# GuildOfWeavers/genSTARK

Measured on AMD Instinct MI355X. Metric: prove() ms + NTT GF(p) elements/sec, MiMC-128 2^20 steps, higher is better.
Workload: dtype u128; 1 GPU; MiMC-128 prove(), 2^20 steps, extensionFactor 16, exeQueryCount 48, friQueryCount 64, blake2s256; one independent proof per GPU; evaluation_domain=16777216, ntt_points_per_prove=17827072, ntt_transforms_per_prove=4, proof_bytes=371695

## Files before the change

genstark_amd/csrc/air_mimc.hip:

```cpp
#include "common.h"
#include "host_field.h"

__global__ void k_mimc_constraints(const fe *__restrict__ p, uint64_t nc, uint64_t shift, const fe *__restrict__ k, uint64_t klen,
                                   fe *__restrict__ out) {
    for (uint64_t j = blockIdx.x * (uint64_t)blockDim.x + threadIdx.x; j < nc; j += (uint64_t)gridDim.x * blockDim.x) {
        uint64_t jn = j + shift;
        if (jn >= nc) jn -= nc;
        fe x = p[j], nx = p[jn];
        fe x3 = fe_mul(fe_mul(x, x), x);
        out[j] = fe_sub(nx, fe_add(x3, k[j % klen]));
    }
}

#define GS_MIMC_COMP_MAX_PERIOD 32
#define GS_MIMC_COMP_MAX_ROOTS 4
struct MimcCompArgs {
    fe qz[GS_MIMC_COMP_MAX_PERIOD];
    fe bt[GS_MIMC_COMP_MAX_PERIOD];
    fe lt[GS_MIMC_COMP_MAX_PERIOD];
    fe ipoly[GS_MIMC_COMP_MAX_ROOTS];
    uint64_t root[GS_MIMC_COMP_MAX_ROOTS];
    fe x_last;
};
__global__ void k_mimc_composition(const fe *__restrict__ p, uint64_t n, uint64_t shift, const fe *__restrict__ k, uint64_t klen,
                                   const fe *__restrict__ tw_lo, const fe *__restrict__ tw_hi, int log_lo, int logn, const fe *__restrict__ u,
                                   MimcCompArgs a, uint32_t period, uint32_t nroots, int with_lc, fe *__restrict__ out) {
    __shared__ fe qz[GS_MIMC_COMP_MAX_PERIOD], bt[GS_MIMC_COMP_MAX_PERIOD], lt[GS_MIMC_COMP_MAX_PERIOD];
    if (threadIdx.x < period) { qz[threadIdx.x] = a.qz[threadIdx.x]; bt[threadIdx.x] = a.bt[threadIdx.x]; lt[threadIdx.x] = a.lt[threadIdx.x]; }
    __syncthreads();
    for (uint64_t i = blockIdx.x * (uint64_t)blockDim.x + threadIdx.x; i < n; i += (uint64_t)gridDim.x * blockDim.x) {
        fe x = tw_lo[i & ((1ull << log_lo) - 1)];
        if (logn > log_lo) x = fe_mul(x, tw_hi[i >> log_lo]);
        const fe pi = p[i], pn = p[(i + shift) & (n - 1)];
        const fe q = fe_sub(pn, fe_add(fe_mul(fe_mul(pi, pi), pi), k[i % klen]));
        const fe d = fe_mul(fe_mul(q, fe_sub(x, a.x_last)), qz[i & (period - 1)]);
        fe iv = a.ipoly[nroots - 1];
        for (int c = (int)nroots - 2; c >= 0; c--) iv = fe_add(fe_mul(iv, x), a.ipoly[c]);
        fe b = fe_mul(fe_sub(pi, iv), bt[i & (period - 1)]);
        for (uint32_t r = 0; r < nroots; r++) b = fe_mul(b, u[(i + n - a.root[r]) & (n - 1)]);
        fe r = fe_add(d, b);
        if (with_lc) r = fe_add(r, fe_mul(pi, lt[i & (period - 1)]));
        out[i] = r;
    }
}

#define GS_MIMC_CHUNK_BODY(STEP)                                                                                \
    for (uint64_t i = base; i < end; i++) {                                                                    \
        t[i] = hf_mimc_out(x);                                      \
        x = STEP(x, rc[ri]);                                   \
        if (++ri == nrc) ri = 0;                                                                               \
    }                                                                                                          \
    *ri_io = ri;                                                                                               \
    return x;
static hfe mimc_chunk_generic(hfe *t, hfe x, const hfe *rc, uint32_t nrc, uint32_t *ri_io, uint64_t base, uint64_t end) {
    uint32_t ri = *ri_io;
    GS_MIMC_CHUNK_BODY(hf_mimc_step_weak)
}
#if defined(__x86_64__) && !defined(__HIP_DEVICE_COMPILE__) && !defined(GS_SMALL_Q) && !defined(GS_WIDE_BITS)
#define GS_MIMC_CHUNK_V3 1
__attribute__((target("arch=x86-64-v3,tune=znver5"))) static hfe mimc_chunk_v3(hfe *t, hfe x, const hfe *rc, uint32_t nrc, uint32_t *ri_io, uint64_t base,
                                                                               uint64_t end) {
    uint32_t ri = *ri_io;
    GS_MIMC_CHUNK_BODY(hf_cube_add_rows)
}
#endif
extern "C" {

int gs_mimc_trace(gs_ctx *c, const gs_elt *seed, const uint8_t *rc_host, uint32_t nrc, uint64_t steps, void *out) {
    if (!c || !seed || !rc_host || !out) return GS_ERR_ARG;
    if (!nrc || !steps) return gs_fail(c, GS_ERR_ARG, "mimc_trace: empty");
    std::vector<hfe> rc(nrc);
    for (uint32_t i = 0; i < nrc; i++) rc[i] = hf_load(rc_host + GS_ELT * i);
    int rcode = gs_trace_begin(c, steps * GS_ELT);
    if (rcode) return rcode;
    hfe *t = (hfe *)c->h_trace;
    hfe x = hf_load(seed);
    uint32_t ri = 0;
    const uint64_t CHUNK = 1ull << 16;
#ifdef GS_MIMC_CHUNK_V3
    static const bool v3 = __builtin_cpu_supports("avx2") && __builtin_cpu_supports("bmi2") && __builtin_cpu_supports("fma");
#else
    const bool v3 = false;
#endif
    for (uint64_t base = 0; base < steps; base += CHUNK) {
        const uint64_t end = base + CHUNK < steps ? base + CHUNK : steps;
#ifdef GS_MIMC_CHUNK_V3
        if (v3) x = mimc_chunk_v3(t, x, rc.data(), nrc, &ri, base, end);
        else
#endif
            x = mimc_chunk_generic(t, x, rc.data(), nrc, &ri, base, end);
        (void)v3;
        GS_HIP(c, hipMemcpyAsync((uint8_t *)out + base * GS_ELT, t + base, (end - base) * GS_ELT, hipMemcpyHostToDevice, c->stream));
    }
    return gs_trace_end(c);
}

int gs_mimc_constraints(gs_ctx *c, const void *p_comp, uint64_t nc, uint64_t shift, const void *k_table, uint64_t klen, void *out) {
    if (!c || !p_comp || !k_table || !out) return GS_ERR_ARG;
    if (!nc || !klen) return gs_fail(c, GS_ERR_ARG, "mimc_constraints: empty");
    hipLaunchKernelGGL(k_mimc_constraints, dim3(gs_grid(nc)), dim3(256), 0, c->stream, (const fe *)p_comp, nc, shift % nc,
                       (const fe *)k_table, klen, (fe *)out);
    GS_LAUNCH_CHECK(c);
    return GS_OK;
}

int gs_mimc_composition(gs_ctx *c, const void *p_eval, uint64_t n, uint64_t steps, const gs_elt *omega, const void *k_table, uint64_t klen,
                        const uint8_t *coeffs_host, uint64_t q_inc, uint64_t b_inc, const uint8_t *ipoly_host, const uint64_t *root_index_host,
                        uint32_t nroots, const uint8_t *lc_coeffs_host, void *out) {
    if (!c || !p_eval || !omega || !k_table || !coeffs_host || !ipoly_host || !root_index_host || !out) return GS_ERR_ARG;
    if (!gs_is_pow2(n) || !gs_is_pow2(steps) || steps > n || !klen) return gs_fail(c, GS_ERR_ARG, "mimc_composition: bad sizes");
    const uint64_t period = n / steps;
    if (period > GS_MIMC_COMP_MAX_PERIOD || nroots == 0 || nroots > GS_MIMC_COMP_MAX_ROOTS)
        return gs_fail(c, GS_ERR_UNSUPPORTED, "mimc_composition: n / steps <= %d and 1..%d assertions", GS_MIMC_COMP_MAX_PERIOD, GS_MIMC_COMP_MAX_ROOTS);
    if (q_inc % steps || b_inc % steps) return gs_fail(c, GS_ERR_ARG, "mimc_composition: degree increments must be multiples of the trace length");
    const fe w = fe_from_bytes(omega);
    const fe *lo, *hi, *u;
    int log_lo;
    int rc = gs_plan_pow_tables(c, w, n, &lo, &hi, &log_lo);
    if (!rc) rc = gs_plan_inverse_table(c, w, n, &u);
    if (rc) return rc;
    const fe d0 = fe_from_bytes(coeffs_host), d1 = fe_from_bytes(coeffs_host + GS_ELT), b0 = fe_from_bytes(coeffs_host + 2 * GS_ELT),
             b1 = fe_from_bytes(coeffs_host + 3 * GS_ELT);
    const fe l0 = lc_coeffs_host ? fe_from_bytes(lc_coeffs_host) : fe_zero(), l1 = lc_coeffs_host ? fe_from_bytes(lc_coeffs_host + GS_ELT) : fe_zero();
    MimcCompArgs a;
    uint64_t ksum = 0;
    for (uint32_t r = 0; r < GS_MIMC_COMP_MAX_ROOTS; r++) {
        a.root[r] = r < nroots ? root_index_host[r] & (n - 1) : 0;
        a.ipoly[r] = r < nroots ? fe_from_bytes(ipoly_host + GS_ELT * r) : fe_zero();
        if (r < nroots) ksum = (ksum + a.root[r]) & (n - 1);
    }
    const fe scale = gs_memo_pow(c, w, (n - ksum) & (n - 1));
    const std::vector<fe> &tab = gs_memo(c, gs_memo_key("mimc_comp").add(w).add(n).add(steps).add(q_inc).add(b_inc), [&](std::vector<fe> &t) {
        const fe g = fe_pow_u64(w, steps);
        const fe gq = fe_pow_u64(g, (q_inc / steps) % period), gb = fe_pow_u64(g, (b_inc / steps) % period);
        fe gj = fe_one(), gqj = fe_one(), gbj = fe_one();
        for (uint64_t j = 0; j < period; j++) {
            t.push_back(fe_inv(fe_sub(gj, fe_one())));
            t.push_back(gqj);
            t.push_back(gbj);
            gj = fe_mul(gj, g); gqj = fe_mul(gqj, gq); gbj = fe_mul(gbj, gb);
        }
        t.push_back(fe_pow_u64(w, (steps - 1) * period));
    });
    for (uint64_t j = 0; j < GS_MIMC_COMP_MAX_PERIOD; j++) {
        if (j < period) {
            a.qz[j] = fe_mul(fe_add(d0, fe_mul(d1, tab[3 * j + 1])), tab[3 * j]);
            a.bt[j] = fe_mul(fe_add(b0, fe_mul(b1, tab[3 * j + 2])), scale);
            a.lt[j] = fe_add(l0, fe_mul(l1, tab[3 * j + 2]));
        } else {
            a.qz[j] = a.bt[j] = a.lt[j] = fe_zero();
        }
    }
    a.x_last = tab[3 * period];
    gs_traffic(c, 2 * n * GS_ELT, n, "k_mimc_composition");
    hipLaunchKernelGGL(k_mimc_composition, dim3(gs_grid(n)), dim3(256), 0, c->stream, (const fe *)p_eval, n, period, (const fe *)k_table, klen, lo, hi,
                       log_lo, gs_log2(n), u, a, (uint32_t)period, nroots, lc_coeffs_host ? 1 : 0, (fe *)out);
    GS_LAUNCH_CHECK(c);
    return GS_OK;
}

}
```

genstark_amd/csrc/common.h:

```cpp
#pragma once
#include <hip/hip_runtime.h>
#include <stdint.h>
#include <stdio.h>
#include <stdarg.h>
#include <string.h>

#include <array>

#include <map>
#include <mutex>
#include <string>
#include <vector>

#include "../../include/gstark.h"
#if defined(GS_SMALL_Q)
#include "gf_small.h"
#elif defined(GS_WIDE_BITS)
#include "gf_wide.h"
#else
#include "gf128.h"
#endif

#if defined(GF_RUNTIME_MODULUS)
typedef int (*gs_rt_push_fn)(void);
// ... 61 lines not shown
    int up_half = 0;
    hipEvent_t up_done[2] = {};
    bool up_pending[2] = {false, false};
};

int gs_fail(gs_ctx *c, int code, const char *fmt, ...);

static inline void gs_traffic(gs_ctx *c, uint64_t bytes, uint64_t units, const char *fmt, ...) __attribute__((format(printf, 4, 5)));
static inline void gs_traffic(gs_ctx *c, uint64_t bytes, uint64_t units, const char *fmt, ...) {
    if (!c->traffic_on) return;
    char name[64];
    va_list ap;
    va_start(ap, fmt);
    vsnprintf(name, sizeof name, fmt, ap);
    va_end(ap);
    auto &e = c->traffic[name];
    e[0] += 1; e[1] += bytes; e[2] += units;
}

struct gs_memo_key {
    std::string k;
    explicit gs_memo_key(const char *tag) : k(tag) {}
    gs_memo_key &add(const void *p, size_t n) { k.append((const char *)p, n); return *this; }
    gs_memo_key &add(uint64_t v) { return add(&v, sizeof v); }
    gs_memo_key &add(const fe &v) { return add(&v, sizeof v); }
};
template <class Build>
static inline const std::vector<fe> &gs_memo(gs_ctx *c, const gs_memo_key &key, Build build) {
    auto it = c->scalar_memo.find(key.k);
    if (it == c->scalar_memo.end()) {
        if (c->scalar_memo.size() > 1024) c->scalar_memo.clear();
        it = c->scalar_memo.emplace(key.k, std::vector<fe>()).first;
        build(it->second);
    }
    return it->second;
}
static inline fe gs_memo_pow(gs_ctx *c, const fe &w, uint64_t e) {
    return gs_memo(c, gs_memo_key("pow").add(w).add(e), [&](std::vector<fe> &t) { t.push_back(fe_pow_u64(w, e)); })[0];
}

#define GS_HIP(c, call)                                                                              \
    do {                                                                                             \
        hipError_t e_ = (call);                                                                      \
        if (e_ != hipSuccess) return gs_fail((c), GS_ERR_DEVICE, "%s: %s", #call, hipGetErrorString(e_)); \
    } while (0)

#define GS_LAUNCH_CHECK(c) GS_HIP(c, hipGetLastError())

static inline bool gs_is_pow2(uint64_t x) { return x && !(x & (x - 1)); }
static inline int gs_log2(uint64_t x) { int l = 0; while ((1ull << l) < x) l++; return l; }

static inline fe fe_from_bytes(const uint8_t *b) { fe r; memcpy(&r, b, sizeof(fe)); return r; }
static inline void fe_to_bytes(uint8_t *b, const fe &v) { memcpy(b, &v, sizeof(fe)); }
static inline fe fe_from_u64(uint64_t v) { return fe_make((uint32_t)v, (uint32_t)(v >> 32), 0, 0); }

int gs_stage_reserve(gs_ctx *c, uint64_t bytes);
int gs_defer_flush(gs_ctx *c);
int gs_push_reserve(gs_ctx *c, uint64_t bytes, void **host);
int gs_push_commit(gs_ctx *c, void *dst, const void *host, uint64_t bytes);
int gs_push(gs_ctx *c, void *dst, const void *host_src, uint64_t bytes);
int gs_readback_reserve(gs_ctx *c, uint32_t bytes, void **slot_dev, unsigned long long **flag_dev, unsigned long long *value, uint64_t *ticket);
int gs_trace_begin(gs_ctx *c, uint64_t bytes);
int gs_trace_end(gs_ctx *c);
int gs_tmp_alloc(gs_ctx *c, uint64_t bytes, void **p);
void gs_tmp_free(gs_ctx *c, void *p);

static inline unsigned gs_grid(uint64_t work_items, unsigned block = 256, unsigned cap = 256 * 8) {
    uint64_t g = (work_items + block - 1) / block;
    if (g < 1) g = 1;
    if (g > cap) g = cap;
    return (unsigned)g;
}

int gs_jit_trace_segments(gs_ctx *c, const uint32_t *code, uint32_t ninstr, const uint32_t *icode, uint32_t init_ninstr, const uint8_t *consts_host,
                          uint32_t nconsts, uint32_t vm_regs, uint32_t registers, const uint64_t *soff, const uint64_t *slen, const uint8_t *statics_host,
                          uint32_t nstatic, const fe *dconst, const fe *dstat, const fe *drows, uint64_t segments, uint64_t seglen, fe *out);
int gs_jit_constraints(gs_ctx *c, const uint32_t *code, uint32_t ninstr, const uint8_t *consts_host, uint32_t nconsts, uint32_t vm_regs,
                       uint32_t registers, const uint64_t *soff, const uint64_t *slen, const fe *dconst, const fe *p, uint64_t nc, uint64_t shift,
                       const fe *statics, fe *out, uint64_t prow, uint64_t pstride);

void gs_plans_destroy(gs_ctx *c);
int gs_plan_pow_tables(gs_ctx *c, const fe &omega, uint64_t n, const fe **tw_lo, const fe **tw_hi, int *log_lo);
int gs_plan_inverse_table(gs_ctx *c, const fe &omega, uint64_t n, const fe **u);
int gs_plan_inverse_table_shifted(gs_ctx *c, const fe &omega, uint64_t n, const fe &shift, const fe **u);
```

genstark_amd/csrc/hash.hip:

```cpp
#include "common.h"

#include "hash_core.h"

template <int ALG, typename Loader>
__device__ __forceinline__ void digest_words16(Loader word16, uint32_t nwords16, uint32_t out[8]) {
    const uint32_t len = nwords16 * 16;
    if (ALG == 1) {
        uint32_t h[8] = {0x6A09E667u ^ 0x01010020u, 0xBB67AE85u, 0x3C6EF372u, 0xA54FF53Au,
                         0x510E527Fu, 0x9B05688Cu, 0x1F83D9ABu, 0x5BE0CD19u};
        const uint32_t nblocks = nwords16 ? (nwords16 + 3) / 4 : 1;
        for (uint32_t blk = 0; blk < nblocks; blk++) {
            uint32_t m[16];
#pragma unroll
            for (int q = 0; q < 4; q++) {
                uint32_t wi = blk * 4 + q;
                uint4 x = wi < nwords16 ? word16(wi) : make_uint4(0, 0, 0, 0);
                m[4 * q] = x.x; m[4 * q + 1] = x.y; m[4 * q + 2] = x.z; m[4 * q + 3] = x.w;
            }
            const bool last = blk == nblocks - 1;
            b2s_compress(h, m, last ? len : (blk + 1) * 64, last);
        }
#pragma unroll
        for (int i = 0; i < 8; i++) out[i] = h[i];
    } else {
// ... 10 lines not shown
                w[4 * q] = bswap32(x.x); w[4 * q + 1] = bswap32(x.y); w[4 * q + 2] = bswap32(x.z); w[4 * q + 3] = bswap32(x.w);
            }
            if (blk == nblocks - 1) { w[14] = 0; w[15] = len * 8; }
            sha256_compress(h, w);
        }
#pragma unroll
        for (int i = 0; i < 8; i++) out[i] = bswap32(h[i]);
    }
}

__device__ __forceinline__ void store_digest(uint4 *out, uint64_t i, const uint32_t d[8]) {
    out[2 * i] = make_uint4(d[0], d[1], d[2], d[3]);
    out[2 * i + 1] = make_uint4(d[4], d[5], d[6], d[7]);
}

struct HashPtrArgs {
    const uint4 *v[GS_MAX_COMBINE];
};

template <int ALG>
__global__ void k_hash_merge_rows(HashPtrArgs va, uint32_t count, uint64_t n, uint4 *__restrict__ out) {
    for (uint64_t i = blockIdx.x * (uint64_t)blockDim.x + threadIdx.x; i < n; i += (uint64_t)gridDim.x * blockDim.x) {
        uint32_t d[8];
        digest_words16<ALG>([&](uint32_t w) { return va.v[w / GS_EW][i * GS_EW + w % GS_EW]; }, count * GS_EW, d);
        store_digest(out, i, d);
    }
}
template <int ALG>
__global__ void k_hash_merge_rows_table(const uint4 *const *__restrict__ tab, uint32_t count, uint64_t n, uint4 *__restrict__ out) {
    for (uint64_t i = blockIdx.x * (uint64_t)blockDim.x + threadIdx.x; i < n; i += (uint64_t)gridDim.x * blockDim.x) {
        uint32_t d[8];
        digest_words16<ALG>([&](uint32_t w) { return tab[w / GS_EW][i * GS_EW + w % GS_EW]; }, count * GS_EW, d);
        store_digest(out, i, d);
    }
}
template <int ALG>
__global__ void k_hash_merge_rows1(const uint4 *__restrict__ v, uint64_t n, uint4 *__restrict__ out) {
    for (uint64_t i = blockIdx.x * (uint64_t)blockDim.x + threadIdx.x; i < n; i += (uint64_t)gridDim.x * blockDim.x) {
        uint32_t d[8];
        digest_words16<ALG>([&](uint32_t w) { return v[i * GS_EW + w]; }, GS_EW, d);
        store_digest(out, i, d);
    }
}
template <int ALG>
__global__ void k_hash_values(const uint4 *__restrict__ buf, uint32_t w16, uint64_t count, uint4 *__restrict__ out) {
    for (uint64_t i = blockIdx.x * (uint64_t)blockDim.x + threadIdx.x; i < count; i += (uint64_t)gridDim.x * blockDim.x) {
        const uint4 *p = buf + i * w16;
        uint32_t d[8];
        digest_words16<ALG>([&](uint32_t w) { return p[w]; }, w16, d);
        store_digest(out, i, d);
    }
}
template <int ALG>
__global__ void k_hash_values64(const uint4 *__restrict__ buf, uint64_t count, uint4 *__restrict__ out) {
    for (uint64_t i = blockIdx.x * (uint64_t)blockDim.x + threadIdx.x; i < count; i += (uint64_t)gridDim.x * blockDim.x) {
        const uint4 *p = buf + i * 4;
        uint4 x0 = p[0], x1 = p[1], x2 = p[2], x3 = p[3];
        uint32_t d[8];
        digest_words16<ALG>([&](uint32_t w) { return w == 0 ? x0 : (w == 1 ? x1 : (w == 2 ? x2 : x3)); }, 4, d);
        store_digest(out, i, d);
    }
}
template <int ALG, int SRC>
__device__ __forceinline__ void first_layer_digest(const HashPtrArgs &va, uint32_t count, const uint4 *__restrict__ child, uint64_t i, uint32_t d[8]) {
    if constexpr (SRC == 0) {
        const uint4 *p = child + 4 * i;
        const uint4 x0 = p[0], x1 = p[1], x2 = p[2], x3 = p[3];
        digest_words16<ALG>([&](uint32_t w) { return w == 0 ? x0 : (w == 1 ? x1 : (w == 2 ? x2 : x3)); }, 4, d);
    } else if constexpr (SRC == 1) {
        const uint4 *p = va.v[0] + i * GS_EW;
        digest_words16<ALG>([&](uint32_t w) { return p[w]; }, GS_EW, d);
    } else {
        digest_words16<ALG>([&](uint32_t w) { return va.v[w / GS_EW][i * GS_EW + w % GS_EW]; }, count * GS_EW, d);
    }
}
template <int ALG>
__device__ __forceinline__ void merge_digests(const uint32_t l[8], const uint32_t r[8], uint32_t d[8]) {
    const uint4 x0 = make_uint4(l[0], l[1], l[2], l[3]), x1 = make_uint4(l[4], l[5], l[6], l[7]);
    const uint4 x2 = make_uint4(r[0], r[1], r[2], r[3]), x3 = make_uint4(r[4], r[5], r[6], r[7]);
    digest_words16<ALG>([&](uint32_t w) { return w == 0 ? x0 : (w == 1 ? x1 : (w == 2 ? x2 : x3)); }, 4, d);
}

#define GS_MERKLE_MAX_LV 4
template <int ALG, int SRC>
__global__ __launch_bounds__(256) void k_merkle_fused(HashPtrArgs va, uint32_t count, const uint4 *__restrict__ child, uint64_t groups, int lv,
                                                      uint4 *__restrict__ outA, uint4 *__restrict__ nodes, uint64_t wA) {
    __shared__ uint32_t pending[GS_MERKLE_MAX_LV - 1][8][256];
    const int K = 1 << (lv - 1), tid = threadIdx.x;
    for (uint64_t g = blockIdx.x * (uint64_t)256 + tid; g < groups; g += (uint64_t)gridDim.x * 256) {
        for (int k = 0; k < K; k++) {
            uint64_t idx = g * K + k;
            uint32_t cur[8];
            first_layer_digest<ALG, SRC>(va, count, child, idx, cur);
            store_digest(outA, idx, cur);
            int h = 0;
            for (; (k >> h) & 1; h++) {
                uint32_t l[8];
#pragma unroll
                for (int w = 0; w < 8; w++) l[w] = pending[h][w][tid];
                merge_digests<ALG>(l, cur, cur);
                idx >>= 1;
                store_digest(nodes, (wA >> (h + 1)) + idx, cur);
            }
            if (h < lv - 1) {
#pragma unroll
                for (int w = 0; w < 8; w++) pending[h][w][tid] = cur[w];
            }
        }
    }
}

struct RootTail {
    uint4 *slot;
    unsigned long long *flag;
    unsigned long long value;
    fe *point;
};
__device__ __forceinline__ fe prng_point(const uint32_t *seed);

#define GS_MERKLE_CHUNK 1024
#define GS_MERKLE_SUBTREE_THREADS 1024
template <int ALG>
__device__ __forceinline__ void subtree_levels(uint4 *sh, uint32_t first_m, uint64_t wl, uint64_t offset, uint4 *__restrict__ nodes) {
    for (uint32_t m = first_m; m >= 1; m >>= 1, wl >>= 1) {
        bool done = false;
        if constexpr (ALG == 1) {
            if (m <= blockDim.x / 4) {
                if (threadIdx.x < 4 * m) {
                    const uint32_t i = threadIdx.x >> 2, l = threadIdx.x & 3u, s = m + i;
                    uint32_t *w = reinterpret_cast<uint32_t *>(sh);
                    uint32_t lo, hi;
                    b2s_node_quad(w + 16 * s, (int)l, lo, hi);
                    w[8 * s + l] = lo;
                    w[8 * s + 4 + l] = hi;
                    uint32_t *g = reinterpret_cast<uint32_t *>(nodes) + 8 * (wl + offset * m + i);
                    g[l] = lo;
                    g[4 + l] = hi;
                }
                done = true;
            }
        }
        if (!done) {
            for (uint32_t i = threadIdx.x; i < m; i += blockDim.x) {
                const uint32_t s = m + i;
                const uint4 x0 = sh[4 * s], x1 = sh[4 * s + 1], x2 = sh[4 * s + 2], x3 = sh[4 * s + 3];
                uint32_t d[8];
                digest_words16<ALG>([&](uint32_t k) { return k == 0 ? x0 : (k == 1 ? x1 : (k == 2 ? x2 : x3)); }, 4, d);
                sh[2 * s] = make_uint4(d[0], d[1], d[2], d[3]);
                sh[2 * s + 1] = make_uint4(d[4], d[5], d[6], d[7]);
                store_digest(nodes, wl + offset * m + i, d);
            }
        }
        __syncthreads();
    }
}

template <int ALG, int SRC>
__global__ __launch_bounds__(GS_MERKLE_SUBTREE_THREADS) void k_merkle_subtree(HashPtrArgs va, uint32_t count, const uint4 *__restrict__ layerA, uint4 *__restrict__ outA,
                                                        uint4 *__restrict__ nodes, uint64_t wA, uint32_t chunk, RootTail tail, unsigned int *counter) {
    __shared__ uint4 sh[4 * GS_MERKLE_CHUNK];
    const uint64_t base = (uint64_t)blockIdx.x * chunk;
    for (uint32_t i = threadIdx.x; i < chunk; i += blockDim.x) {
        if constexpr (SRC == 0) {
            sh[2 * (chunk + i)] = layerA[2 * (base + i)];
            sh[2 * (chunk + i) + 1] = layerA[2 * (base + i) + 1];
        } else {
            uint32_t d[8];
            first_layer_digest<ALG, SRC>(va, count, nullptr, base + i, d);
            store_digest(outA, base + i, d);
            sh[2 * (chunk + i)] = make_uint4(d[0], d[1], d[2], d[3]);
            sh[2 * (chunk + i) + 1] = make_uint4(d[4], d[5], d[6], d[7]);
        }
    }
    __syncthreads();
    subtree_levels<ALG>(sh, chunk / 2, wA >> 1, blockIdx.x, nodes);
    bool at_root = chunk == wA;
    if (counter && gridDim.x > 1) {
        __shared__ int last_sh;
        const uint32_t G = gridDim.x;
        if (threadIdx.x == 0) {
            __threadfence();
            last_sh = atomicAdd(counter, 1u) == G - 1;
            if (last_sh) __threadfence();
        }
        __syncthreads();
        if (!last_sh) return;
        for (uint32_t i = threadIdx.x; i < G; i += blockDim.x) {
            sh[2 * (G + i)] = nodes[2 * (G + (uint64_t)i)];
            sh[2 * (G + i) + 1] = nodes[2 * (G + (uint64_t)i) + 1];
        }
        if (threadIdx.x == 0) atomicExch(counter, 0u);
        __syncthreads();
        subtree_levels<ALG>(sh, G / 2, G >> 1, 0, nodes);
        at_root = true;
    }
    if (at_root && threadIdx.x == 0) {
        nodes[0] = make_uint4(0, 0, 0, 0);
        nodes[1] = make_uint4(0, 0, 0, 0);
        if (tail.slot) {
            tail.slot[0] = sh[2];
            tail.slot[1] = sh[3];
            __threadfence_system();
            __hip_atomic_store(tail.flag, tail.value, __ATOMIC_RELEASE, __HIP_MEMORY_SCOPE_SYSTEM);
        }
        if (tail.point) {
            const uint4 r0 = sh[2], r1 = sh[3];
            const uint32_t seed[8] = {r0.x, r0.y, r0.z, r0.w, r1.x, r1.y, r1.z, r1.w};
            *tail.point = prng_point(seed);
        }
    }
}

#define GS_FRI_MAX_LAYERS 16
static int arrival_counters(gs_ctx *c, unsigned int **counters) {
    if (!c->fri_points) {
        int rc = gs_alloc(c, (GS_FRI_MAX_LAYERS + 1) * GS_ELT + 64, &c->fri_points);
        if (rc) return rc;
        GS_HIP(c, hipMemsetAsync((uint8_t *)c->fri_points + (GS_FRI_MAX_LAYERS + 1) * GS_ELT, 0, 64, c->stream));
    }
    *counters = (unsigned int *)((uint8_t *)c->fri_points + (GS_FRI_MAX_LAYERS + 1) * GS_ELT);
    return GS_OK;
}

static inline uint64_t hash_blocks(int alg, uint64_t bytes) { return alg == 1 ? (bytes + 63) / 64 : (bytes + 9 + 63) / 64; }
#define GS_MERKLE_SUBW (1ull << 15)
template <int ALG>
static int merkle_run(gs_ctx *c, int src, const HashPtrArgs &va, uint32_t count, const void *leaves_in, void *leaves_out, uint64_t n, uint4 *nd,
                      const RootTail *root_tail = nullptr) {
    const RootTail none = {nullptr, nullptr, 0, nullptr};
    auto tail_for = [&](uint64_t width, uint32_t chunk) { return root_tail && (width == chunk || width / chunk <= GS_MERKLE_CHUNK) ? *root_tail : none; };
    const uint32_t CHUNK_X = 256;
    unsigned int *counters = nullptr;
    if (n > CHUNK_X) {
        int rc = arrival_counters(c, &counters);
        if (rc) return rc;
        counters += 1;
    }
    const dim3 blk(256), sub_blk(GS_MERKLE_SUBTREE_THREADS);
    uint64_t w = n;
    const uint4 *cur = (const uint4 *)leaves_in;
    if (src != 0) {
        uint4 *lo = (uint4 *)leaves_out;
        if (n > GS_MERKLE_SUBW) {
            int lv = 1;
            const int maxlv = src == 2 ? 2 : GS_MERKLE_MAX_LV;
            while (lv < maxlv && (n >> lv) >= GS_MERKLE_SUBW) lv++;
            const uint64_t groups = n >> (lv - 1);
            {
                const uint64_t above = n - (n >> (lv - 1));
                gs_traffic(c, n * ((uint64_t)count * GS_ELT + 32) + above * 32, n * hash_blocks(ALG, (uint64_t)count * GS_ELT) + above, "k_merkle_fused<%d, %d>", ALG, src);
            }
            if (src == 1) hipLaunchKernelGGL((k_merkle_fused<ALG, 1>), dim3(gs_grid(groups)), blk, 0, c->stream, va, count, nullptr, groups, lv, lo, nd, n);
            else hipLaunchKernelGGL((k_merkle_fused<ALG, 2>), dim3(gs_grid(groups)), blk, 0, c->stream, va, count, nullptr, groups, lv, lo, nd, n);
            w = n >> (lv - 1);
            cur = lv == 1 ? lo : nd + 2 * w;
        } else {
            const uint32_t chunk = (uint32_t)(n <= CHUNK_X ? n : CHUNK_X);
            gs_traffic(c, n * ((uint64_t)count * GS_ELT + 32) + n * 32, n * hash_blocks(ALG, (uint64_t)count * GS_ELT) + n - 1, "k_merkle_subtree<%d, %d>", ALG, src);
            if (src == 1) hipLaunchKernelGGL((k_merkle_subtree<ALG, 1>), dim3((unsigned)(n / chunk)), sub_blk, 0, c->stream, va, count, nullptr, lo, nd, n, chunk, tail_for(n, chunk), counters);
            else hipLaunchKernelGGL((k_merkle_subtree<ALG, 2>), dim3((unsigned)(n / chunk)), sub_blk, 0, c->stream, va, count, nullptr, lo, nd, n, chunk, tail_for(n, chunk), counters);
            GS_LAUNCH_CHECK(c);
            return GS_OK;
        }
    }
    while (w > GS_MERKLE_SUBW) {
        int lv = 1;
        while (lv < GS_MERKLE_MAX_LV && (w >> (lv + 1)) >= GS_MERKLE_SUBW) lv++;
#ifdef GS_NTT_EXPERIMENTS
        if (const char *e = getenv("GSTARK_MERKLE_NODE_MIN_GROUPS")) {
            const int K = atoi(e);
            lv = 1;
            while (lv < GS_MERKLE_MAX_LV && (w >> (lv + 1)) >= GS_MERKLE_SUBW) lv++;
            while (lv > 1 && (w >> lv) < (1ull << K)) lv--;
        }
#endif
        const uint64_t groups = w >> lv;
        gs_traffic(c, w * 32 + (w - (w >> lv)) * 32, w - (w >> lv), "k_merkle_fused<%d, 0>", ALG);
        hipLaunchKernelGGL((k_merkle_fused<ALG, 0>), dim3(gs_grid(groups)), blk, 0, c->stream, va, 0u, cur, groups, lv, nd + 2 * (w / 2), nd, w / 2);
        w >>= lv;
        cur = nd + 2 * w;
    }
    while (w > 1) {
        const uint32_t chunk = (uint32_t)(w <= CHUNK_X ? w : (w / CHUNK_X <= GS_MERKLE_CHUNK ? CHUNK_X : GS_MERKLE_CHUNK));
        gs_traffic(c, w * 32 + (w - 1) * 32, w - 1, "k_merkle_subtree<%d, 0>", ALG);
        hipLaunchKernelGGL((k_merkle_subtree<ALG, 0>), dim3((unsigned)(w / chunk)), sub_blk, 0, c->stream, va, 0u, cur, nullptr, nd, w, chunk, tail_for(w, chunk), counters);
        w /= chunk;
        cur = nd + 2 * w;
        if (counters && w <= GS_MERKLE_CHUNK) break;
    }
    GS_LAUNCH_CHECK(c);
    return GS_OK;
}

template <int ALG>
static int hash_values_launch(gs_ctx *c, const void *buf, uint64_t value_size, uint64_t count, void *out) {
    if (!count) return GS_OK;
    if (value_size == 64)
        hipLaunchKernelGGL(k_hash_values64<ALG>, dim3(gs_grid(count)), dim3(256), 0, c->stream, (const uint4 *)buf, count, (uint4 *)out);
    else
        hipLaunchKernelGGL(k_hash_values<ALG>, dim3(gs_grid(count)), dim3(256), 0, c->stream, (const uint4 *)buf,
                           (uint32_t)(value_size / 16), count, (uint4 *)out);
    GS_LAUNCH_CHECK(c);
    return GS_OK;
}

static int check_alg(gs_ctx *c, gs_hash_alg alg) {
    if (alg != GS_HASH_SHA256 && alg != GS_HASH_BLAKE2S256) return gs_fail(c, GS_ERR_ARG, "unknown hash algorithm %d", (int)alg);
    return GS_OK;
}

__device__ __forceinline__ fe prng_point(const uint32_t *seed);
__global__ void k_prng_point(const uint32_t *__restrict__ seed, fe *__restrict__ out) {
    if (threadIdx.x || blockIdx.x) return;
    *out = prng_point(seed);
}
__device__ __forceinline__ fe prng_point(const uint32_t *seed) {
    uint32_t h[8] = {0x6a09e667u, 0xbb67ae85u, 0x3c6ef372u, 0xa54ff53au, 0x510e527fu, 0x9b05688cu, 0x1f83d9abu, 0x5be0cd19u};
    uint32_t w[16];
#pragma unroll
    for (int i = 0; i < 8; i++) w[i] = bswap32(seed[i]);
    w[8] = 0x80000000u;
#pragma unroll
    for (int i = 9; i < 15; i++) w[i] = 0;
    w[15] = 256;
    sha256_compress(h, w);
#if !defined(GS_SMALL_Q) && !defined(GS_WIDE_BITS)
    const uint32_t r[8] = {h[7], h[6], h[5], h[4], h[3], h[2], h[1], h[0]};
    return fe_reduce_wide(r);
#else
    fe x = fe_zero();
    const fe b = fe_make(256u, 0u, 0u, 0u);
    for (int i = 0; i < 8; i++)
        for (int k = 3; k >= 0; k--) x = fe_add(fe_mul(x, b), fe_make((h[i] >> (8 * k)) & 0xFFu, 0u, 0u, 0u));
    return x;
#endif
}
int gs_prng_point_dev(gs_ctx *c, const void *seed32_dev, fe *out_dev) {
    if (((uintptr_t)seed32_dev) & 3) return gs_fail(c, GS_ERR_ARG, "prng_point: the seed must be 4-byte aligned");
    hipLaunchKernelGGL(k_prng_point, dim3(1), dim3(64), 0, c->stream, (const uint32_t *)seed32_dev, out_dev);
    GS_LAUNCH_CHECK(c);
    return GS_OK;
}


#define GS_FRI_CH 256
#define GS_FRI_THREADS (4 * GS_FRI_CH)
#define GS_FRI_ONE_LAUNCH_LEAVES (1ull << 15)
struct FriLayerDesc {
    const fe *column;
    fe *next;
    uint4 *leaves, *nodes;
    fe *point_out;
    uint4 *slot;
    unsigned long long *flag;
    unsigned long long value;
    uint64_t rows, step;
};
struct FriLayersArgs {
    FriLayerDesc layer[GS_FRI_MAX_LAYERS];
    uint32_t first, count;
    const fe *point_in;
// ... 301 lines not shown
```

genstark_amd/csrc/ntt.hip:

```cpp
#include <stdlib.h>

#include "common.h"

#if !defined(GS_SMALL_Q) && !defined(GS_WIDE_BITS)
#define GS_NTT_LAZY 1
#include "gf128_lazy.h"
struct alignas(32) lz8 { int32_t l[8]; };
#endif

struct NttPlan {
    fe omega;
    uint64_t n = 0;
    int logn = 0, log_lo = 0;
    fe *tw_lo = nullptr;
    fe *tw_hi = nullptr;
    int npass = 0;
    int L[4] = {0, 0, 0, 0};
    fe *wR[4] = {nullptr, nullptr, nullptr, nullptr};
    fe *twp[4] = {nullptr, nullptr, nullptr, nullptr};
    fe w16[8];
    fe *inv_table = nullptr;
    std::map<std::string, fe *> inv_table_shifted;
#ifdef GS_NTT_LAZY
    lzw *wtab = nullptr;
// ... 645 lines not shown
    }
    if (p->logn >= 8) {
        int np = (p->logn + 7) / 8, base = p->logn / np, extra = p->logn % np;
        p->npass = np;
        fe w16 = fe_pow_u64(omega, n / 16), cur = fe_one();
        for (int i = 0; i < 8; i++) { p->w16[i] = cur; cur = fe_mul(cur, w16); }
#ifdef GS_NTT_LAZY
        {
            lzw host[8];
            for (int i = 1; i < 8; i++) lz_wform(p->w16[i], host[i - 1]);
            lz_wform(fe_inv(fe_from_u64(n)), host[7]);
            if ((rc = gs_alloc(c, sizeof host, &q))) { delete p; return rc; }
            p->wtab = (lzw *)q;
            if (hipMemcpyAsync(p->wtab, host, sizeof host, hipMemcpyHostToDevice, c->stream) != hipSuccess ||
                hipStreamSynchronize(c->stream) != hipSuccess) {
                delete p;
                return gs_fail(c, GS_ERR_DEVICE, "ntt: twiddle upload failed");
            }
        }
#endif
#ifdef GS_NTT_LAZY
        if ((rc = gs_alloc(c, (1ull << p->log_lo) * GS_ELT, &q))) { delete p; return rc; }
        p->tw_loR = (fe *)q;
        hipLaunchKernelGGL(k_scale_table, dim3(gs_grid(1ull << p->log_lo)), dim3(256), 0, c->stream, p->tw_lo, p->tw_loR, 1ull << p->log_lo, lz_mont_r());
#endif
        uint64_t Ns_acc = 1;
        for (int i = 0; i < np; i++) {
            p->L[i] = base + (i < extra ? 1 : 0);
            uint64_t R = 1ull << p->L[i];
            if (i > 0 && Ns_acc * R <= max_pass_twiddle_entries()) {
#if !defined(GS_NTT_LAZY) || defined(GS_NTT_EXPERIMENTS)
                if ((rc = gs_alloc(c, Ns_acc * R * GS_ELT, &q))) { delete p; return rc; }
                p->twp[i] = (fe *)q;
                hipLaunchKernelGGL(k_build_pass_twiddles, dim3(gs_grid(Ns_acc * R)), dim3(256), 0, c->stream, p->twp[i], Ns_acc, R,
                                   n / (Ns_acc * R), p->tw_lo, p->tw_hi, p->log_lo, p->logn, fe_one(), 0);
#endif
#ifdef GS_NTT_LAZY
                if ((rc = gs_alloc(c, Ns_acc * R * GS_ELT, &q))) { delete p; return rc; }
                p->twpR[i] = (fe *)q;
                hipLaunchKernelGGL(k_build_pass_twiddles, dim3(gs_grid(Ns_acc * R)), dim3(256), 0, c->stream, p->twpR[i], Ns_acc, R,
                                   n / (Ns_acc * R), p->tw_lo, p->tw_hi, p->log_lo, p->logn, lz_mont_r(), 1);
#endif
            }
            Ns_acc *= R;
            if (R > 16) {
                for (int k = 0; k < i; k++)
                    if (p->L[k] == p->L[i]) p->wR[i] = p->wR[k];
                if (!p->wR[i]) {
                    if ((rc = gs_alloc(c, R * GS_ELT, &q))) { delete p; return rc; }
                    p->wR[i] = (fe *)q;
                    if ((rc = gs_power_series_dev(c, fe_pow_u64(omega, n / R), R, p->wR[i]))) { delete p; return rc; }
                }
#ifdef GS_NTT_LAZY
                for (int k = 0; k < i; k++)
                    if (p->L[k] == p->L[i]) p->wRz[i] = p->wRz[k];
                if (!p->wRz[i]) {
                    if ((rc = gs_alloc(c, R * sizeof(lz8), &q))) { delete p; return rc; }
                    p->wRz[i] = (lz8 *)q;
                    hipLaunchKernelGGL(k_build_lz_table, dim3(gs_grid(R)), dim3(256), 0, c->stream, p->wR[i], p->wRz[i], R, lz_mont_r(), 1);
                }
#endif
            }
        }
    }
    c->plans[key] = p;
    *out = p;
    return GS_OK;
}

void gs_plans_destroy(gs_ctx *c) {
    for (auto &kv : c->plans) delete kv.second;
    c->plans.clear();
}

int gs_plan_pow_tables(gs_ctx *c, const fe &omega, uint64_t n, const fe **tw_lo, const fe **tw_hi, int *log_lo) {
    NttPlan *p;
    int rc = plan_get(c, omega, n, &p);
    if (rc) return rc;
    *tw_lo = p->tw_lo;
    *tw_hi = p->tw_hi;
    *log_lo = p->log_lo;
    return GS_OK;
}

__global__ void k_omega_minus_one(const fe *__restrict__ tw_lo, const fe *__restrict__ tw_hi, int log_lo, int logn, uint64_t n,
                                  fe shift, int has_shift, fe *__restrict__ out) {
    for (uint64_t i = blockIdx.x * (uint64_t)blockDim.x + threadIdx.x; i < n; i += (uint64_t)gridDim.x * blockDim.x) {
        fe x = pow_lookup(tw_lo, tw_hi, log_lo, logn, i);
        if (has_shift) x = fe_mul(x, shift);
        out[i] = fe_sub(x, fe_one());
    }
}

int gs_vec_inv_dev(gs_ctx *c, const fe *a, uint64_t n, fe *out);

int gs_plan_inverse_table(gs_ctx *c, const fe &omega, uint64_t n, const fe **u) {
    NttPlan *p;
    int rc = plan_get(c, omega, n, &p);
    if (rc) return rc;
    if (!p->inv_table) {
        void *q = nullptr, *t = nullptr;
        if ((rc = gs_alloc(c, n * GS_ELT, &q))) return rc;
        if ((rc = gs_tmp_alloc(c, n * GS_ELT, &t))) { gs_free(c, q); return rc; }
        hipLaunchKernelGGL(k_omega_minus_one, dim3(gs_grid(n)), dim3(256), 0, c->stream, p->tw_lo, p->tw_hi, p->log_lo, p->logn, n, fe_one(), 0, (fe *)t);
        rc = gs_vec_inv_dev(c, (const fe *)t, n, (fe *)q);
        gs_tmp_free(c, t);
        if (rc) { gs_free(c, q); return rc; }
        p->inv_table = (fe *)q;
    }
    *u = p->inv_table;
    return GS_OK;
}
int gs_plan_inverse_table_shifted(gs_ctx *c, const fe &omega, uint64_t n, const fe &shift, const fe **u) {
    if (fe_eq(shift, fe_one())) return gs_plan_inverse_table(c, omega, n, u);
    NttPlan *p;
    int rc = plan_get(c, omega, n, &p);
    if (rc) return rc;
    const std::string key = plan_key(shift, 0);
    auto it = p->inv_table_shifted.find(key);
    if (it == p->inv_table_shifted.end()) {
        void *q = nullptr, *t = nullptr;
        if ((rc = gs_alloc(c, n * GS_ELT, &q))) return rc;
        if ((rc = gs_tmp_alloc(c, n * GS_ELT, &t))) { gs_free(c, q); return rc; }
        hipLaunchKernelGGL(k_omega_minus_one, dim3(gs_grid(n)), dim3(256), 0, c->stream, p->tw_lo, p->tw_hi, p->log_lo, p->logn, n, shift, 1, (fe *)t);
        rc = gs_vec_inv_dev(c, (const fe *)t, n, (fe *)q);
        gs_tmp_free(c, t);
        if (rc) { gs_free(c, q); return rc; }
        it = p->inv_table_shifted.emplace(key, (fe *)q).first;
    }
    *u = it->second;
    return GS_OK;
}

template <int LB>
static void launch_pass(gs_ctx *c, const fe *in, fe *out, const PassArgs &a, uint32_t rows) {
    constexpr int RB = 1 << LB, R = 16 * RB;
    const int Wj = 1 << a.logWj;
    const uint64_t tiles = (a.n / R) / Wj;
    const bool need_lds = (RB > 1) || (a.logNs == 0);
    const size_t lds = need_lds ? (size_t)Wj * (R + 1) * GS_ELT : 0;
    if (lds > 64 * 1024)
        (void)hipFuncSetAttribute(reinterpret_cast<const void *>(k_ntt_pass<LB>), hipFuncAttributeMaxDynamicSharedMemorySize, 160 * 1024);
    hipLaunchKernelGGL(k_ntt_pass<LB>, dim3((unsigned)tiles, rows), dim3(RB * Wj), lds, c->stream, in, out, a);
}


#ifdef GS_NTT_LAZY
template <int LB>
static void launch_pass_lz(gs_ctx *c, const fe *in, fe *out, const LzPassArgs &a, uint32_t rows) {
    constexpr int RB = 1 << LB, R = 16 * RB;
    const int Wj = 1 << a.logWj;
    const uint64_t tiles = (a.n / R) / Wj;
    const bool first = a.logNs == 0;
    size_t lds = 0;
    if (RB > 1) lds = (size_t)5 * 4 * R * Wj;
    if (first) { const size_t tr = (size_t)Wj * (R + 1) * sizeof(fe); if (tr > lds) lds = tr; }
    gs_traffic(c, (uint64_t)rows * ((first ? a.in_len : a.n) + a.n) * GS_ELT, (uint64_t)rows * a.n, "k_ntt_pass_lz<%d, %d>", LB, first ? 0 : (a.twp ? 1 : 2));
    if (first) hipLaunchKernelGGL((k_ntt_pass_lz<LB, 0>), dim3((unsigned)tiles, rows), dim3(RB * Wj), lds, c->stream, in, out, a);
    else if (a.twp) hipLaunchKernelGGL((k_ntt_pass_lz<LB, 1>), dim3((unsigned)tiles, rows), dim3(RB * Wj), lds, c->stream, in, out, a);
    else hipLaunchKernelGGL((k_ntt_pass_lz<LB, 2>), dim3((unsigned)tiles, rows), dim3(RB * Wj), lds, c->stream, in, out, a);
}

template <int LB>
static void launch_pass_wave(gs_ctx *c, const fe *in, fe *out, const LzPassArgs &a, uint32_t rows) {
    constexpr int RB = 1 << LB, R = 16 * RB, Wj = 64 >> LB;
    const uint64_t tiles = (a.n / R) / Wj;
// ... 219 lines not shown
```

Before: 1.663 billion elements/s.

## Use lazy Montgomery arithmetic in MiMC composition and templatize Merkle fused levels

The MiMC composition kernel now runs its field arithmetic in a lazy-reduction Montgomery representation. Host-side period constants are pre-scaled by powers of R, and an R-scaled low twiddle table is used so results come out in standard form, cutting full reductions per element. Separately, the fused Merkle kernel is templated on level count so that for ALG 1 pending digests stay in registers via a compile-time climb instead of shared memory, with the inner loop unrolled. This relies on a tw_loR plan member existing and on the Montgomery scaling being exactly right, and it adds code size and register pressure.

```diff
diff --git a/genstark_amd/csrc/air_mimc.hip b/genstark_amd/csrc/air_mimc.hip
--- a/genstark_amd/csrc/air_mimc.hip
+++ b/genstark_amd/csrc/air_mimc.hip
@@ -22,6 +22,10 @@
     uint64_t root[GS_MIMC_COMP_MAX_ROOTS];
     fe x_last;
 };
+#if !defined(GS_SMALL_Q) && !defined(GS_WIDE_BITS)
+#define GS_MIMC_COMP_LAZY 1
+#include "gf128_lazy.h"
+#endif
 __global__ void k_mimc_composition(const fe *__restrict__ p, uint64_t n, uint64_t shift, const fe *__restrict__ k, uint64_t klen,
                                    const fe *__restrict__ tw_lo, const fe *__restrict__ tw_hi, int log_lo, int logn, const fe *__restrict__ u,
                                    MimcCompArgs a, uint32_t period, uint32_t nroots, int with_lc, fe *__restrict__ out) {
@@ -29,6 +33,22 @@
     if (threadIdx.x < period) { qz[threadIdx.x] = a.qz[threadIdx.x]; bt[threadIdx.x] = a.bt[threadIdx.x]; lt[threadIdx.x] = a.lt[threadIdx.x]; }
     __syncthreads();
     for (uint64_t i = blockIdx.x * (uint64_t)blockDim.x + threadIdx.x; i < n; i += (uint64_t)gridDim.x * blockDim.x) {
+#ifdef GS_MIMC_COMP_LAZY
+        const lzk K = lzk_make();
+        lz x = lz_unpack(tw_lo[i & ((1ull << log_lo) - 1)]);
+        if (logn > log_lo) x = lz_mul_vm(lz_unpack(tw_hi[i >> log_lo]), x, K);
+        const lz pi = lz_unpack(p[i]), pn = lz_unpack(p[(i + shift) & (n - 1)]);
+        const lz q = lz_sub(lz_sub(pn, lz_mul_v(lz_sqr(pi, K), pi, K)), lz_unpack(k[i % klen]));
+        const lz xl = lz_norm(lz_sub(x, lz_unpack(a.x_last)));
+        const lz d = lz_mul_vm(lz_mul_vm(q, xl, K), lz_unpack(qz[i & (period - 1)]), K);
+        lz iv = lz_unpack(a.ipoly[nroots - 1]);
+        for (int c = (int)nroots - 2; c >= 0; c--) iv = lz_add(lz_mul_v(iv, x, K), lz_unpack(a.ipoly[c]));
+        lz b = lz_mul_vm(lz_sub(pi, iv), lz_unpack(bt[i & (period - 1)]), K);
+        for (uint32_t r = 0; r < nroots; r++) b = lz_mul_vm(b, lz_unpack(u[(i + n - a.root[r]) & (n - 1)]), K);
+        lz r = lz_add(d, b);
+        if (with_lc) r = lz_add(r, lz_mul_vm(pi, lz_unpack(lt[i & (period - 1)]), K));
+        out[i] = lz_pack(r);
+#else
         fe x = tw_lo[i & ((1ull << log_lo) - 1)];
         if (logn > log_lo) x = fe_mul(x, tw_hi[i >> log_lo]);
         const fe pi = p[i], pn = p[(i + shift) & (n - 1)];
@@ -41,6 +61,7 @@
         fe r = fe_add(d, b);
         if (with_lc) r = fe_add(r, fe_mul(pi, lt[i & (period - 1)]));
         out[i] = r;
+#endif
     }
 }
 
@@ -142,11 +163,20 @@
         }
         t.push_back(fe_pow_u64(w, (steps - 1) * period));
     });
+#ifdef GS_MIMC_COMP_LAZY
+    const fe R = lz_mont_r(), R2 = lz_mont_r2();
+    fe rb = R;
+    for (uint32_t r = 0; r < nroots; r++) rb = fe_mul(rb, R);
+    const fe sq = R2, sb = fe_mul(scale, rb), sl = R;
+    if (gs_log2(n) > log_lo && (rc = gs_plan_pow_table_lo_r(c, w, n, &lo))) return rc;
+#else
+    const fe sq = fe_one(), sb = scale, sl = fe_one();
+#endif
     for (uint64_t j = 0; j < GS_MIMC_COMP_MAX_PERIOD; j++) {
         if (j < period) {
-            a.qz[j] = fe_mul(fe_add(d0, fe_mul(d1, tab[3 * j + 1])), tab[3 * j]);
-            a.bt[j] = fe_mul(fe_add(b0, fe_mul(b1, tab[3 * j + 2])), scale);
-            a.lt[j] = fe_add(l0, fe_mul(l1, tab[3 * j + 2]));
+            a.qz[j] = fe_mul(fe_mul(fe_add(d0, fe_mul(d1, tab[3 * j + 1])), tab[3 * j]), sq);
+            a.bt[j] = fe_mul(fe_add(b0, fe_mul(b1, tab[3 * j + 2])), sb);
+            a.lt[j] = fe_mul(fe_add(l0, fe_mul(l1, tab[3 * j + 2])), sl);
         } else {
             a.qz[j] = a.bt[j] = a.lt[j] = fe_zero();
         }
diff --git a/genstark_amd/csrc/common.h b/genstark_amd/csrc/common.h
--- a/genstark_amd/csrc/common.h
+++ b/genstark_amd/csrc/common.h
@@ -167,4 +167,7 @@
 void gs_plans_destroy(gs_ctx *c);
 int gs_plan_pow_tables(gs_ctx *c, const fe &omega, uint64_t n, const fe **tw_lo, const fe **tw_hi, int *log_lo);
 int gs_plan_inverse_table(gs_ctx *c, const fe &omega, uint64_t n, const fe **u);
+#if !defined(GS_SMALL_Q) && !defined(GS_WIDE_BITS)
+int gs_plan_pow_table_lo_r(gs_ctx *c, const fe &omega, uint64_t n, const fe **tw_loR);
+#endif
 int gs_plan_inverse_table_shifted(gs_ctx *c, const fe &omega, uint64_t n, const fe &shift, const fe **u);
diff --git a/genstark_amd/csrc/hash.hip b/genstark_amd/csrc/hash.hip
--- a/genstark_amd/csrc/hash.hip
+++ b/genstark_amd/csrc/hash.hip
@@ -116,31 +116,67 @@
 }
 
 #define GS_MERKLE_MAX_LV 4
-template <int ALG, int SRC>
-__global__ __launch_bounds__(256) void k_merkle_fused(HashPtrArgs va, uint32_t count, const uint4 *__restrict__ child, uint64_t groups, int lv,
+template <int LV>
+struct MerklePending {
+    uint32_t r[LV > 1 ? LV - 1 : 1][8];
+};
+template <int LV, int H>
+__device__ __forceinline__ void merkle_climb(MerklePending<LV> &pend, uint32_t cur[8], int k, uint64_t idx, uint4 *__restrict__ nodes, uint64_t wA) {
+    if constexpr (H < LV - 1) {
+        if (!((k >> H) & 1)) {
+#pragma unroll
+            for (int w = 0; w < 8; w++) pend.r[H][w] = cur[w];
+            return;
+        }
+        merge_digests<1>(pend.r[H], cur, cur);
+        idx >>= 1;
+        store_digest(nodes, (wA >> (H + 1)) + idx, cur);
+        merkle_climb<LV, H + 1>(pend, cur, k, idx, nodes, wA);
+    }
+}
+template <int ALG, int SRC, int LV>
+__global__ __launch_bounds__(256) void k_merkle_fused(HashPtrArgs va, uint32_t count, const uint4 *__restrict__ child, uint64_t groups,
                                                       uint4 *__restrict__ outA, uint4 *__restrict__ nodes, uint64_t wA) {
-    __shared__ uint32_t pending[GS_MERKLE_MAX_LV - 1][8][256];
-    const int K = 1 << (lv - 1), tid = threadIdx.x;
+    constexpr int K = 1 << (LV - 1), KU = ALG == 1 && LV <= 2 ? K : 1;
+    __shared__ uint32_t pending_sh[ALG == 1 || LV == 1 ? 1 : LV - 1][8][ALG == 1 || LV == 1 ? 1 : 256];
+    const int tid = threadIdx.x;
     for (uint64_t g = blockIdx.x * (uint64_t)256 + tid; g < groups; g += (uint64_t)gridDim.x * 256) {
+        MerklePending<LV> pend;
+#pragma unroll KU
         for (int k = 0; k < K; k++) {
             uint64_t idx = g * K + k;
             uint32_t cur[8];
             first_layer_digest<ALG, SRC>(va, count, child, idx, cur);
             store_digest(outA, idx, cur);
-            int h = 0;
-            for (; (k >> h) & 1; h++) {
-                uint32_t l[8];
-#pragma unroll
-                for (int w = 0; w < 8; w++) l[w] = pending[h][w][tid];
-                merge_digests<ALG>(l, cur, cur);
-                idx >>= 1;
-                store_digest(nodes, (wA >> (h + 1)) + idx, cur);
-            }
-            if (h < lv - 1) {
-#pragma unroll
-                for (int w = 0; w < 8; w++) pending[h][w][tid] = cur[w];
-            }
-        }
+            if constexpr (ALG == 1) {
+                merkle_climb<LV, 0>(pend, cur, k, idx, nodes, wA);
+            } else {
+                int h = 0;
+                for (; (k >> h) & 1; h++) {
+                    uint32_t l[8];
+#pragma unroll
+                    for (int w = 0; w < 8; w++) l[w] = pending_sh[h][w][tid];
+                    merge_digests<ALG>(l, cur, cur);
+                    idx >>= 1;
+                    store_digest(nodes, (wA >> (h + 1)) + idx, cur);
+                }
+                if (h < LV - 1) {
+#pragma unroll
+                    for (int w = 0; w < 8; w++) pending_sh[h][w][tid] = cur[w];
+                }
+            }
+        }
+    }
+}
+template <int ALG, int SRC>
+static void launch_merkle_fused(gs_ctx *c, int lv, const HashPtrArgs &va, uint32_t count, const uint4 *child, uint64_t groups, uint4 *outA,
+                                uint4 *nodes, uint64_t wA) {
+    const dim3 grid(gs_grid(groups)), blk(256);
+    switch (lv) {
+    case 1: hipLaunchKernelGGL((k_merkle_fused<ALG, SRC, 1>), grid, blk, 0, c->stream, va, count, child, groups, outA, nodes, wA); break;
+    case 2: hipLaunchKernelGGL((k_merkle_fused<ALG, SRC, 2>), grid, blk, 0, c->stream, va, count, child, groups, outA, nodes, wA); break;
+    case 3: hipLaunchKernelGGL((k_merkle_fused<ALG, SRC, 3>), grid, blk, 0, c->stream, va, count, child, groups, outA, nodes, wA); break;
+    default: hipLaunchKernelGGL((k_merkle_fused<ALG, SRC, 4>), grid, blk, 0, c->stream, va, count, child, groups, outA, nodes, wA); break;
     }
 }
 
@@ -270,7 +306,7 @@
         if (rc) return rc;
         counters += 1;
     }
-    const dim3 blk(256), sub_blk(GS_MERKLE_SUBTREE_THREADS);
+    const dim3 sub_blk(GS_MERKLE_SUBTREE_THREADS);
     uint64_t w = n;
     const uint4 *cur = (const uint4 *)leaves_in;
     if (src != 0) {
@@ -284,8 +320,8 @@
                 const uint64_t above = n - (n >> (lv - 1));
                 gs_traffic(c, n * ((uint64_t)count * GS_ELT + 32) + above * 32, n * hash_blocks(ALG, (uint64_t)count * GS_ELT) + above, "k_merkle_fused<%d, %d>", ALG, src);
             }
-            if (src == 1) hipLaunchKernelGGL((k_merkle_fused<ALG, 1>), dim3(gs_grid(groups)), blk, 0, c->stream, va, count, nullptr, groups, lv, lo, nd, n);
-            else hipLaunchKernelGGL((k_merkle_fused<ALG, 2>), dim3(gs_grid(groups)), blk, 0, c->stream, va, count, nullptr, groups, lv, lo, nd, n);
+            if (src == 1) launch_merkle_fused<ALG, 1>(c, lv, va, count, nullptr, groups, lo, nd, n);
+            else launch_merkle_fused<ALG, 2>(c, lv, va, count, nullptr, groups, lo, nd, n);
             w = n >> (lv - 1);
             cur = lv == 1 ? lo : nd + 2 * w;
         } else {
@@ -310,7 +346,7 @@
 #endif
         const uint64_t groups = w >> lv;
         gs_traffic(c, w * 32 + (w - (w >> lv)) * 32, w - (w >> lv), "k_merkle_fused<%d, 0>", ALG);
-        hipLaunchKernelGGL((k_merkle_fused<ALG, 0>), dim3(gs_grid(groups)), blk, 0, c->stream, va, 0u, cur, groups, lv, nd + 2 * (w / 2), nd, w / 2);
+        launch_merkle_fused<ALG, 0>(c, lv, va, 0u, cur, groups, nd + 2 * (w / 2), nd, w / 2);
         w >>= lv;
         cur = nd + 2 * w;
     }
diff --git a/genstark_amd/csrc/ntt.hip b/genstark_amd/csrc/ntt.hip
--- a/genstark_amd/csrc/ntt.hip
+++ b/genstark_amd/csrc/ntt.hip
@@ -751,6 +751,16 @@
     *log_lo = p->log_lo;
     return GS_OK;
 }
+
+#ifdef GS_NTT_LAZY
+int gs_plan_pow_table_lo_r(gs_ctx *c, const fe &omega, uint64_t n, const fe **tw_loR) {
+    NttPlan *p;
+    int rc = plan_get(c, omega, n, &p);
+    if (rc) return rc;
+    *tw_loR = p->tw_loR;
+    return GS_OK;
+}
+#endif
 
 __global__ void k_omega_minus_one(const fe *__restrict__ tw_lo, const fe *__restrict__ tw_hi, int log_lo, int logn, uint64_t n,
                                   fe shift, int has_shift, fe *__restrict__ out) {
```

After: 1.646 billion elements/s (median of 2 runs). 0.99x the previous value.
